# lucidrains/vit-pytorch

Hardware: NVIDIA H100
Metric: images/sec ViT-B/16 224^2 bf16 fwd (higher is better)
Workload: dtype bf16

## Files before the change

### vit_pytorch_b200/csrc/gemm.cu

```cuda
#include "common.cuh"
#include "host_util.h"

namespace b200 {

constexpr int BLOCK_M = 128;
constexpr int BLOCK_K = 64;
constexpr int WGMMA_K = 16;
constexpr int NUM_THREADS = 384;
constexpr int NUM_CONSUMERS = 256;

struct GemmParams {
  int M, N, K;
  int num_m_tiles, num_n_tiles, num_k_blocks;
  int flags;
  __nv_bfloat16* out_bf16;
  float* out_f32;
  long long ldo;
  const float* bias;
  const float* ln_sums;
  int ln_parts;
  int stats_parts;
  int stats_width;
  float ln_inv_dim;
  float ln_eps;
  const float* col_s;
  float* stats_out;
  int rows_per_tile;
  int patch;
  int patch_ght;
  int patch_tiles_per_img;
  int patch_C;
};

template <int BLOCK_N, int STAGES, bool PATCH = false, bool RES = false, bool TMA_OUT = false>
struct GemmSmem {
  static constexpr int A_SLAB = PATCH ? BLOCK_M * 32 : BLOCK_M * BLOCK_K * 2;
  static constexpr int A_BYTES = PATCH ? 4 * A_SLAB : A_SLAB;
  static constexpr int B_BYTES = BLOCK_N * BLOCK_K * 2;
  static constexpr int STAGE_BYTES = A_BYTES + B_BYTES;
  static constexpr int RES_BOX = BLOCK_M * 32 * 4;
  static constexpr int RES_SLAB = 2 * RES_BOX;
  static constexpr int RES_OFFSET = STAGES * STAGE_BYTES;
  static constexpr int OUT_BOX = 64 * 64 * 2;
  static constexpr int OUT_OFFSET = RES_OFFSET + (RES ? 2 * RES_SLAB : 0);
  static constexpr int OUT_BYTES = !TMA_OUT ? 0 : RES ? 2 * OUT_BOX : BLOCK_M * BLOCK_N * 2;
  static constexpr int VEC_OFFSET = OUT_OFFSET + OUT_BYTES;
  static constexpr int VEC_BYTES = (2 * BLOCK_N + 2 * BLOCK_M) * 4;
  static constexpr int BAR_OFFSET = VEC_OFFSET + 2 * VEC_BYTES;
  static constexpr int TOTAL = BAR_OFFSET + (2 * STAGES + 8) * 8;
  static constexpr int DYN_BYTES = TOTAL + 1024;
};

__device__ __forceinline__ void warpgroup_sync(int c) { asm volatile("bar.sync %0, 128;" ::"r"(c + 1) : "memory"); }

template <int BLOCK_N, int STAGES, bool PATCH, bool RES, bool TMA_OUT>
__global__ void __launch_bounds__(NUM_THREADS, 1)
gemm_bf16_kernel(const __grid_constant__ CUtensorMap tmA, const __grid_constant__ CUtensorMap tmB,
                 const __grid_constant__ CUtensorMap tmR, const __grid_constant__ CUtensorMap tmO,
                 const __grid_constant__ CUtensorMap tmF, const GemmParams p) {
  static_assert(!(TMA_OUT && PATCH), "patch tiles have fewer than 128 rows: a 64-row box would overwrite the next one");
  using L = GemmSmem<BLOCK_N, STAGES, PATCH, RES, TMA_OUT>;
  constexpr int NACC = BLOCK_N / 2;
  constexpr int CHUNKS = BLOCK_N / 64;

  extern __shared__ uint8_t smem_raw[];
  uint8_t* smem = smem_raw + ((1024u - (smem_u32(smem_raw) & 1023u)) & 1023u);
  uint64_t* full_bar = reinterpret_cast<uint64_t*>(smem + L::BAR_OFFSET);
  uint64_t* empty_bar = full_bar + STAGES;
  uint64_t* res_full = empty_bar + STAGES;
  uint64_t* res_empty = res_full + 2;
  uint64_t* vec_full = res_empty + 2;
  uint64_t* vec_empty = vec_full + 2;

  const int wg = threadIdx.x >> 7;
  const int num_tiles = p.num_m_tiles * p.num_n_tiles;

  if (threadIdx.x == 0) {
    tma_prefetch_desc(&tmA);
    tma_prefetch_desc(&tmB);
    if (RES) tma_prefetch_desc(&tmR);
    if (TMA_OUT && p.out_bf16) tma_prefetch_desc(&tmO);
    if (TMA_OUT && RES && p.out_f32) tma_prefetch_desc(&tmF);
    for (int s = 0; s < STAGES; ++s) {
      mbar_init(&full_bar[s], 1);
      mbar_init(&empty_bar[s], 2);
    }
    for (int s = 0; s < 2; ++s) {
      mbar_init(&res_full[s], 1);
      mbar_init(&res_empty[s], TMA_OUT ? 2 : NUM_CONSUMERS);
      mbar_init(&vec_full[s], 64);
      mbar_init(&vec_empty[s], NUM_CONSUMERS);
    }
    fence_mbar_init();
  }
  __syncthreads();

  if (wg == 0) {
    setmaxnreg_dec<40>();
    if (threadIdx.x == 0) {
      int stage = 0;
      uint32_t phase = 0;
      for (int tile = blockIdx.x; tile < num_tiles; tile += gridDim.x) {
        const int m_blk = tile / p.num_n_tiles;
        const int n_blk = tile % p.num_n_tiles;
        for (int kb = 0; kb < p.num_k_blocks; ++kb) {
          mbar_wait(&empty_bar[stage], phase ^ 1);
          uint8_t* sa = smem + stage * L::STAGE_BYTES;
          uint8_t* sb = sa + L::A_BYTES;
          if (PATCH) {
            const int img = m_blk / p.patch_tiles_per_img, tin = m_blk % p.patch_tiles_per_img;
            mbar_arrive_expect_tx(&full_bar[stage], p.rows_per_tile * 128 + L::B_BYTES);
#pragma unroll
            for (int j = 0; j < 4; ++j)
              tma_load_5d(sa + j * L::A_SLAB, &tmA, &full_bar[stage], 0, 0, tin * p.patch_ght, (kb & 3) * 4 + j,
                          img * p.patch_C + (kb >> 2));
          } else {
            mbar_arrive_expect_tx(&full_bar[stage], L::STAGE_BYTES);
            tma_load_2d(sa, &tmA, &full_bar[stage], kb * BLOCK_K, m_blk * BLOCK_M);
          }
          tma_load_2d(sb, &tmB, &full_bar[stage], kb * BLOCK_K, n_blk * BLOCK_N);
          if (++stage == STAGES) {
            stage = 0;
            phase ^= 1;
          }
        }
      }
    } else if (RES && threadIdx.x == 32) {
      int it = 0;
      for (int tile = blockIdx.x; tile < num_tiles; tile += gridDim.x) {
        const int n0 = (tile % p.num_n_tiles) * BLOCK_N;
        const int m0 = (tile / p.num_n_tiles) * BLOCK_M;
        const int nslab = min(CHUNKS, (p.N - n0 + 63) / 64);
        for (int q = 0; q < nslab; ++q, ++it) {
          const int buf = it & 1;
          mbar_wait(&res_empty[buf], ((it >> 1) & 1) ^ 1);
          const int c0 = n0 + 64 * q;
          const int nbox = c0 + 32 < p.N ? 2 : 1;
          mbar_arrive_expect_tx(&res_full[buf], nbox * L::RES_BOX);
          uint8_t* slab = smem + L::RES_OFFSET + buf * L::RES_SLAB;
          for (int b = 0; b < nbox; ++b) tma_load_2d(slab + b * L::RES_BOX, &tmR, &res_full[buf], c0 + 32 * b, m0);
        }
      }
    } else if ((threadIdx.x >> 5) >= 2) {
      const int lane = threadIdx.x & 31;
      const bool vec_warp = (threadIdx.x >> 5) == 2;
      int it = 0;
      for (int tile = blockIdx.x; tile < num_tiles; tile += gridDim.x, ++it) {
        const int m_blk = tile / p.num_n_tiles;
        const int n0 = (tile % p.num_n_tiles) * BLOCK_N;
        const int vb = it & 1;
        mbar_wait(&vec_empty[vb], ((it >> 1) & 1) ^ 1);
        float* vbias = reinterpret_cast<float*>(smem + L::VEC_OFFSET + vb * L::VEC_BYTES);
        float* vcs = vbias + BLOCK_N;
        float2* vln = reinterpret_cast<float2*>(vcs + BLOCK_N);
        if (vec_warp) {
#pragma unroll
          for (int i = lane; i < BLOCK_N; i += 32) {
            const int col = n0 + i;
            vbias[i] = (p.flags & B200VIT_EPI_BIAS) && col < p.N ? p.bias[col] : 0.f;
            vcs[i] = (p.flags & B200VIT_EPI_LNFOLD) && col < p.N ? p.col_s[col] : 0.f;
          }
        } else if (p.flags & B200VIT_EPI_LNFOLD) {
          float s1[BLOCK_M / 32], s2[BLOCK_M / 32];
          bool ok[BLOCK_M / 32];
#pragma unroll
          for (int k = 0; k < BLOCK_M / 32; ++k) {
            const int tr = lane + 32 * k;
            ok[k] = m_blk * p.rows_per_tile + tr < p.M && tr < p.rows_per_tile;
            s1[k] = s2[k] = 0.f;
          }
#pragma unroll 1
          for (int i = 0; i < p.ln_parts; ++i)
#pragma unroll
            for (int k = 0; k < BLOCK_M / 32; ++k)
              if (ok[k]) {
                const size_t row = (size_t)m_blk * p.rows_per_tile + lane + 32 * k;
                const float2 ss = *reinterpret_cast<const float2*>(p.ln_sums + 2 * (row * p.ln_parts + i));
                s1[k] += ss.x;
                s2[k] += ss.y;
              }
#pragma unroll
          for (int k = 0; k < BLOCK_M / 32; ++k) vln[lane + 32 * k] = make_float2(s1[k], s2[k]);
        }
        mbar_arrive(&vec_full[vb]);
      }
    }
    return;
  }

  setmaxnreg_inc<232>();
  const int c = wg - 1;
  const int t = threadIdx.x & 127;
  const int warp = t >> 5, lane = t & 31;
  const int flags = p.flags;
  const bool vec_ok = (p.ldo & 1) == 0;
  int stage = 0;
  uint32_t phase = 0;
  int slab_it = 0;
  int pend_slab = -1;
  uint8_t* const stg_wg = smem + L::OUT_OFFSET + c * (RES ? L::OUT_BOX : 64 * BLOCK_N * 2);
  float acc[NACC];

  for (int tile = blockIdx.x, it = 0; tile < num_tiles; tile += gridDim.x, ++it) {
    const int m_blk = tile / p.num_n_tiles;
    const int n_blk = tile % p.num_n_tiles;

    int prev_stage = -1;
    for (int kb = 0; kb < p.num_k_blocks; ++kb) {
      mbar_wait(&full_bar[stage], phase);
      const uint32_t sa = smem_u32(smem + stage * L::STAGE_BYTES);
      const uint32_t sb = sa + L::A_BYTES;
      const uint64_t bdesc = make_wgmma_desc(sb, 1024, WGMMA_SW128);
      wgmma_fence();
#pragma unroll
      for (int k = 0; k < BLOCK_K / WGMMA_K; ++k) {
        const uint64_t ad = PATCH ? make_wgmma_desc(sa + k * L::A_SLAB + c * 64 * 32, 256, WGMMA_SW32)
                                  : make_wgmma_desc(sa + c * 64 * 128, 1024, WGMMA_SW128) + 2 * k;
        if constexpr (BLOCK_N == 256) wgmma_m64n256k16(acc, ad, bdesc + 2 * k, (kb | k) != 0);
        else wgmma_m64n128k16(acc, ad, bdesc + 2 * k, (kb | k) != 0);
      }
      wgmma_commit();
      if (TMA_OUT && kb == 0 && t == 0) {
        tma_store_wait_read<0>();
        if (RES && pend_slab >= 0) mbar_arrive(&res_empty[pend_slab]);
        pend_slab = -1;
      }
      wgmma_wait<1>();
      if (prev_stage >= 0 && t == 0) mbar_arrive(&empty_bar[prev_stage]);
      prev_stage = stage;
      if (++stage == STAGES) {
        stage = 0;
        phase ^= 1;
      }
    }
    wgmma_wait<0>();
    fence_regs(acc);
    if (t == 0) mbar_arrive(&empty_bar[prev_stage]);
    if (TMA_OUT && !RES) warpgroup_sync(c);

    const int tr0 = c * 64 + warp * 16 + (lane >> 2);
    const int vb = it & 1;
    mbar_wait(&vec_full[vb], (it >> 1) & 1);
    const float* vbias = reinterpret_cast<const float*>(smem + L::VEC_OFFSET + vb * L::VEC_BYTES);
    const float* vcs = vbias + BLOCK_N;
    const float2* vln = reinterpret_cast<const float2*>(vcs + BLOCK_N);
    float mu[2] = {0.f, 0.f}, rstd[2] = {1.f, 1.f};
    int row[2];
    bool row_ok[2];
#pragma unroll
    for (int h = 0; h < 2; ++h) {
      const int tr = tr0 + 8 * h;
      row[h] = m_blk * p.rows_per_tile + tr;
      row_ok[h] = row[h] < p.M && tr < p.rows_per_tile;
      if ((flags & B200VIT_EPI_LNFOLD) && row_ok[h]) {
        const float2 ss = vln[tr];
        const float s1 = ss.x, s2 = ss.y;
        mu[h] = s1 * p.ln_inv_dim;
        const float var = fmaxf(s2 * p.ln_inv_dim - mu[h] * mu[h], 0.f);
        rstd[h] = rsqrtf(var + p.ln_eps);
      }
    }
    float st_sum[2][CHUNKS], st_sq[2][CHUNKS];
#pragma unroll
    for (int q = 0; q < CHUNKS; ++q) st_sum[0][q] = st_sum[1][q] = st_sq[0][q] = st_sq[1][q] = 0.f;

    const int n0 = n_blk * BLOCK_N;
    const int nslab = RES ? min(CHUNKS, (p.N - n0 + 63) / 64) : 0;
    const int res_off = tr0 * 128 + (lane & 1) * 8;
    const int res_xor = ((lane & 3) >> 1) ^ (lane >> 2);
    const int stg_off = (tr0 - 64 * c) * 128 + 4 * (lane & 3);
    uint32_t pks[8][2] = {};
#pragma unroll
    for (int j = 0; j < BLOCK_N / 8; ++j) {
      const int pc = 8 * j + 2 * (lane & 3);
      const int col = n0 + pc;
      if (RES && j % 8 == 0 && j / 8 < nslab) mbar_wait(&res_full[slab_it & 1], (slab_it >> 1) & 1);
      uint8_t* slab = smem + L::RES_OFFSET + (slab_it & 1) * L::RES_SLAB + ((j % 8) / 4) * L::RES_BOX + res_off;
      uint8_t* stg = stg_wg + (RES ? 0 : (j / 8) * L::OUT_BOX) + stg_off + (((j % 8) ^ (lane >> 2)) << 4);
      const bool pair = vec_ok && col + 1 < p.N;
      float b0 = 0.f, b1 = 0.f, s0 = 0.f, s1 = 0.f;
      if (flags & B200VIT_EPI_BIAS) {
        const float2 bb = *reinterpret_cast<const float2*>(vbias + pc);
        b0 = bb.x;
        b1 = bb.y;
      }
      if (flags & B200VIT_EPI_LNFOLD) {
        const float2 ss = *reinterpret_cast<const float2*>(vcs + pc);
        s0 = ss.x;
        s1 = ss.y;
      }
#pragma unroll
      for (int h = 0; h < 2; ++h) {
        if (!row_ok[h] || col >= p.N) continue;
        float v0 = acc[4 * j + 2 * h], v1 = acc[4 * j + 2 * h + 1];
        if (flags & (B200VIT_EPI_LNFOLD | B200VIT_EPI_BIAS)) {
          const bool fold = (flags & B200VIT_EPI_LNFOLD) != 0;
          const float k = -rstd[h] * mu[h];
          const float c0 = fold ? fmaf(k, s0, b0) : b0, c1 = fold ? fmaf(k, s1, b1) : b1;
          const float rs = fold ? rstd[h] : 1.0f;
          v0 = fmaf(v0, rs, c0);
          v1 = fmaf(v1, rs, c1);
        }
        if (flags & B200VIT_EPI_GELU) gelu_erf2(v0, v1);
        const size_t o = (size_t)row[h] * p.ldo + col;
        float2* rp = reinterpret_cast<float2*>(slab + h * 8 * 128 + ((((j % 4) * 2) ^ res_xor) << 4));
        float2 rr = make_float2(0.f, 0.f);
        if (RES) rr = *rp;
        float r0 = 0.f, r1 = 0.f;
        if (TMA_OUT) {
          if (RES) {
            v0 += rr.x;
            v1 += rr.y;
            if (p.out_f32) *rp = make_float2(v0, v1);
          }
          const uint32_t pk = pack_bf16x2(v0, v1);
          if (RES) pks[j % 8][h] = pk;
          else *reinterpret_cast<uint32_t*>(stg + h * 8 * 128) = pk;
          r0 = __uint_as_float(pk << 16);
          r1 = __uint_as_float(pk & 0xFFFF0000u);
        } else if (pair) {
          if (RES) {
            v0 += rr.x;
            v1 += rr.y;
          }
          if (p.out_f32) *reinterpret_cast<float2*>(p.out_f32 + o) = make_float2(v0, v1);
          const uint32_t pk = pack_bf16x2(v0, v1);
          if (p.out_bf16) *reinterpret_cast<uint32_t*>(p.out_bf16 + o) = pk;
          r0 = __uint_as_float(pk << 16);
          r1 = __uint_as_float(pk & 0xFFFF0000u);
        } else {
          const float vv[2] = {v0, v1}, res[2] = {rr.x, rr.y};
          float rb[2] = {0.f, 0.f};
          for (int i = 0; i < 2 && col + i < p.N; ++i) {
            float x = vv[i];
            if (RES) x += res[i];
            if (p.out_f32) p.out_f32[o + i] = x;
            const __nv_bfloat16 xb = __float2bfloat16_rn(x);
            if (p.out_bf16) p.out_bf16[o + i] = xb;
            rb[i] = __bfloat162float(xb);
          }
          r0 = rb[0];
          r1 = rb[1];
        }
        if (flags & B200VIT_EPI_STATS) {
          st_sum[h][j / 8] += r0 + r1;
          st_sq[h][j / 8] = fmaf(r0, r0, fmaf(r1, r1, st_sq[h][j / 8]));
        }
      }
      if (RES && j % 8 == 7 && j / 8 < nslab) {
        if constexpr (TMA_OUT) {
          if (t == 0) {
            tma_store_wait_read<0>();
            if (pend_slab >= 0) mbar_arrive(&res_empty[pend_slab]);
            pend_slab = -1;
          }
          warpgroup_sync(c);
          if (p.out_bf16)
#pragma unroll
            for (int jj = 0; jj < 8; ++jj)
#pragma unroll
              for (int h = 0; h < 2; ++h)
                *reinterpret_cast<uint32_t*>(stg_wg + stg_off + ((jj ^ (lane >> 2)) << 4) + h * 8 * 128) = pks[jj][h];
          fence_proxy_async_smem();
          warpgroup_sync(c);
          if (t == 0) {
            const int buf = slab_it & 1, c0 = n0 + 64 * (j / 8), row0 = m_blk * BLOCK_M + 64 * c;
            if (row0 < p.M) {
              const uint8_t* half = smem + L::RES_OFFSET + buf * L::RES_SLAB + c * 64 * 128;
              if (p.out_f32)
                for (int b = 0; b < 2 && c0 + 32 * b < p.N; ++b)
                  tma_store_2d(&tmF, half + b * L::RES_BOX, c0 + 32 * b, row0);
              if (p.out_bf16) tma_store_2d(&tmO, stg_wg, c0, row0);
            }
            tma_store_commit();
            pend_slab = buf;
          }
        } else {
          mbar_arrive(&res_empty[slab_it & 1]);
        }
        ++slab_it;
      }
    }
    mbar_arrive(&vec_empty[vb]);
    if constexpr (TMA_OUT && !RES) {
      fence_proxy_async_smem();
      warpgroup_sync(c);
      if (t == 0) {
        const int row0 = m_blk * BLOCK_M + 64 * c;
        if (row0 < p.M)
          for (int b = 0; b < BLOCK_N / 64 && n0 + 64 * b < p.N; ++b)
            tma_store_2d(&tmO, stg_wg + b * L::OUT_BOX, n0 + 64 * b, row0);
        tma_store_commit();
      }
    }
    if (flags & B200VIT_EPI_STATS) {
#pragma unroll
      for (int h = 0; h < 2; ++h)
#pragma unroll
        for (int q = 0; q < CHUNKS; ++q) {
          st_sum[h][q] += __shfl_xor_sync(0xffffffffu, st_sum[h][q], 1);
          st_sum[h][q] += __shfl_xor_sync(0xffffffffu, st_sum[h][q], 2);
          st_sq[h][q] += __shfl_xor_sync(0xffffffffu, st_sq[h][q], 1);
          st_sq[h][q] += __shfl_xor_sync(0xffffffffu, st_sq[h][q], 2);
        }
      if ((lane & 3) == 0) {
        const int per = p.stats_width / 64;
        const int first = n0 / p.stats_width;
        const int last = (n_blk == p.num_n_tiles - 1) ? p.stats_parts : first + CHUNKS / per;
#pragma unroll
        for (int h = 0; h < 2; ++h) {
          if (!row_ok[h]) continue;
          float* so = p.stats_out + 2 * (size_t)row[h] * p.stats_parts;
          for (int part = first; part < last; ++part) {
            float a = 0.f, b = 0.f;
#pragma unroll
            for (int q = 0; q < CHUNKS; ++q)
              if (first + q / per == part) {
                a += st_sum[h][q];
                b += st_sq[h][q];
              }
            *reinterpret_cast<float2*>(so + 2 * part) = make_float2(a, b);
          }
        }
      }
    }
  }
  if (TMA_OUT && t == 0) tma_store_wait<0>();
}

static std::atomic<int> g_gemm_block_n{0};
void gemm_set_block_n(int v) { g_gemm_block_n = v; }
static std::atomic<int> g_gemm_direct_store{0};
void gemm_set_direct_store(int v) { g_gemm_direct_store = v; }

template <int BLOCK_N, int STAGES, bool PATCH = false, bool RES = false, bool TMA_OUT = false>
static int launch_gemm(const CUtensorMap& tmA, const CUtensorMap& tmB, const CUtensorMap& tmR, const CUtensorMap& tmO,
                       const CUtensorMap& tmF, GemmParams& p, cudaStream_t stream) {
  using L = GemmSmem<BLOCK_N, STAGES, PATCH, RES, TMA_OUT>;
  static_assert(L::DYN_BYTES <= 227 * 1024, "gemm: shared memory budget");
  auto kern = gemm_bf16_kernel<BLOCK_N, STAGES, PATCH, RES, TMA_OUT>;
  B200_ENSURE_SMEM(kern, L::DYN_BYTES);
  if (!p.patch) p.rows_per_tile = BLOCK_M;
  p.num_m_tiles = (p.M + p.rows_per_tile - 1) / p.rows_per_tile;
  p.num_n_tiles = (p.N + BLOCK_N - 1) / BLOCK_N;
  p.num_k_blocks = (p.K + BLOCK_K - 1) / BLOCK_K;
  p.stats_width = p.N > 128 ? 128 : 64;
  const int tiles = p.num_m_tiles * p.num_n_tiles;
  const int grid = tiles < num_sms() ? tiles : num_sms();
  kern<<<grid, NUM_THREADS, L::DYN_BYTES, stream>>>(tmA, tmB, tmR, tmO, tmF, p);
  B200_CHECK_CUDA(cudaGetLastError());
  count_launch();
  return 0;
}

}

extern "C" int b200vit_stats_parts(int N) {
  const int block_n = N > 128 ? 256 : 128;
  return 2 * ((N + block_n - 1) / block_n);
}

extern "C" int b200vit_gemm_bf16(const void* A, int64_t lda, const void* W, int64_t ldw, void* out_bf16,
                                 float* out_f32, int64_t ldo, const float* bias, const float* resid,
                                 const float* ln_sums, int ln_parts, float ln_eps, const float* col_s,
                                 float* stats_out, int M, int N, int K, int flags, void* stream) {
  using namespace b200;
  B200_CHECK_ARG(A && W, "gemm: A/W must not be null");
  B200_CHECK_ARG(out_bf16 || out_f32, "gemm: need at least one output");
  B200_CHECK_ARG(M > 0 && N > 0 && K > 0, "gemm: bad shape M=%d N=%d K=%d", M, N, K);
  B200_CHECK_ARG((reinterpret_cast<uintptr_t>(A) & 15) == 0 && (reinterpret_cast<uintptr_t>(W) & 15) == 0,
                 "gemm: A and W must be 16-byte aligned");
  B200_CHECK_ARG((lda & 7) == 0 && (ldw & 7) == 0 && lda >= K && ldw >= K,
                 "gemm: lda=%lld ldw=%lld must be multiples of 8 and >= K=%d", (long long)lda, (long long)ldw, K);
  B200_CHECK_ARG(ldo >= N, "gemm: ldo=%lld < N=%d", (long long)ldo, N);
  B200_CHECK_ARG(!(flags & B200VIT_EPI_BIAS) || bias, "gemm: EPI_BIAS without bias");
  B200_CHECK_ARG(!(flags & B200VIT_EPI_RESIDUAL) || resid, "gemm: EPI_RESIDUAL without resid");
  B200_CHECK_ARG(!(flags & B200VIT_EPI_RESIDUAL) || (ldo & 3) == 0,
                 "gemm: EPI_RESIDUAL needs ldo=%lld to be a multiple of 4 (16-byte rows for TMA)", (long long)ldo);
  B200_CHECK_ARG(!(flags & B200VIT_EPI_LNFOLD) || (ln_sums && col_s && ln_parts >= 1 && ln_parts <= 64),
                 "gemm: EPI_LNFOLD needs ln_sums, col_s and 1 <= ln_parts <= 64");
  B200_CHECK_ARG(!(flags & B200VIT_EPI_STATS) || stats_out, "gemm: EPI_STATS without stats_out");
  auto al16 = [](const void* q) { return (reinterpret_cast<uintptr_t>(q) & 15) == 0; };
  B200_CHECK_ARG(al16(bias) && al16(resid) && al16(col_s) && al16(out_bf16) && al16(out_f32) && al16(ln_sums),
                 "gemm: epilogue pointers must be 16-byte aligned");

  cudaStream_t st = reinterpret_cast<cudaStream_t>(stream);

  GemmParams p{};
  p.M = M; p.N = N; p.K = K;
  p.flags = flags;
  p.out_bf16 = reinterpret_cast<__nv_bfloat16*>(out_bf16);
  p.out_f32 = out_f32;
  p.ldo = ldo;
  p.bias = bias;
  p.ln_sums = ln_sums;
  p.ln_parts = ln_parts;
  p.stats_parts = b200vit_stats_parts(N);
  p.ln_inv_dim = 1.0f / (float)K;
  p.ln_eps = ln_eps;
  p.col_s = col_s;
  p.stats_out = stats_out;

  const bool res = (flags & B200VIT_EPI_RESIDUAL) != 0;
  const bool tma_ok = !g_gemm_direct_store.load() && ((ldo | N) & 7) == 0 && (res || !out_f32);
  const int force = g_gemm_block_n.load();
  const bool wide = force == 0 ? N > 128 && !(res && tma_ok) : force == 2;
  const uint32_t block_n = wide ? 256 : 128;
  const bool tma_out = tma_ok && !(res && wide);
  CUtensorMap tmA, tmB, tmR{}, tmO{}, tmF{};
  if (tma_out && out_bf16) {
    const uint64_t dims[2] = {(uint64_t)N, (uint64_t)M};
    const uint64_t strides[1] = {(uint64_t)ldo * 2};
    const uint32_t box[2] = {64, 64};
    int rc = encode_tmap_bf16(&tmO, out_bf16, 2, dims, strides, box);
    if (rc) return rc;
  }
  if (tma_out && res && out_f32) {
    const uint64_t dims[2] = {(uint64_t)N, (uint64_t)M};
    const uint64_t strides[1] = {(uint64_t)ldo * 4};
    const uint32_t box[2] = {32, 64};
    int rc = encode_tmap_f32(&tmF, out_f32, 2, dims, strides, box, true);
    if (rc) return rc;
  }
  if (res) {
    const uint64_t dims[2] = {(uint64_t)N, (uint64_t)M};
    const uint64_t strides[1] = {(uint64_t)ldo * 4};
    const uint32_t box[2] = {32, (uint32_t)BLOCK_M};
    int rc = encode_tmap_f32(&tmR, resid, 2, dims, strides, box, true);
    if (rc) return rc;
  }
  {
    const uint64_t dims[2] = {(uint64_t)K, (uint64_t)M};
    const uint64_t strides[1] = {(uint64_t)lda * 2};
    const uint32_t box[2] = {(uint32_t)BLOCK_K, (uint32_t)BLOCK_M};
    int rc = encode_tmap_bf16(&tmA, A, 2, dims, strides, box);
    if (rc) return rc;
  }
  {
    const uint64_t dims[2] = {(uint64_t)K, (uint64_t)N};
    const uint64_t strides[1] = {(uint64_t)ldw * 2};
    const uint32_t box[2] = {(uint32_t)BLOCK_K, block_n};
    int rc = encode_tmap_bf16(&tmB, W, 2, dims, strides, box);
    if (rc) return rc;
  }
  if (tma_out) {
    if (res) return launch_gemm<128, 4, false, true, true>(tmA, tmB, tmR, tmO, tmF, p, st);
    return wide ? launch_gemm<256, 3, false, false, true>(tmA, tmB, tmR, tmO, tmF, p, st)
                : launch_gemm<128, 5, false, false, true>(tmA, tmB, tmR, tmO, tmF, p, st);
  }
  if (wide)
    return res ? launch_gemm<256, 3, false, true>(tmA, tmB, tmR, tmO, tmF, p, st)
               : launch_gemm<256, 4>(tmA, tmB, tmR, tmO, tmF, p, st);
  return res ? launch_gemm<128, 4, false, true>(tmA, tmB, tmR, tmO, tmF, p, st)
             : launch_gemm<128, 6>(tmA, tmB, tmR, tmO, tmF, p, st);
}

extern "C" int b200vit_rmsnorm_heads(void* buf, int64_t ld, const float* gamma, int T, int nheads, int dh, void* stream);
extern "C" int b200vit_layernorm_heads(void* buf, int64_t ld, const float* gamma, int T, int nheads, int dh, float eps,
                                       void* stream);

extern "C" int b200vit_gemm_headnorm_bf16(const void* A, int64_t lda, const void* W, int64_t ldw, void* out_bf16,
                                          int64_t ldo, const float* bias, const float* ln_sums, int ln_parts,
                                          float ln_eps, const float* col_s, const float* head_gamma, int norm_heads,
                                          int dh, float head_eps, int M, int N, int K, int flags, void* stream) {
  using namespace b200;
  B200_CHECK_ARG(out_bf16 && head_gamma, "gemm_headnorm: null pointer");
  B200_CHECK_ARG(head_width_ok(dh), "gemm_headnorm: dim_head=%d not supported by this build (32, 64, 80 or 128)", dh);
  B200_CHECK_ARG(norm_heads > 0 && norm_heads * dh <= N, "gemm_headnorm: %d heads do not fit N=%d", norm_heads, N);
  B200_CHECK_ARG((flags & ~(B200VIT_EPI_BIAS | B200VIT_EPI_LNFOLD | B200VIT_EPI_HEADLN)) == 0,
                 "gemm_headnorm: unsupported flags %d", flags);
  const bool hln = (flags & B200VIT_EPI_HEADLN) != 0;
  B200_CHECK_ARG((reinterpret_cast<uintptr_t>(head_gamma) & 15) == 0, "gemm_headnorm: head_gamma must be 16-byte aligned");
  int rc = b200vit_gemm_bf16(A, lda, W, ldw, out_bf16, nullptr, ldo, bias, nullptr, ln_sums, ln_parts, ln_eps, col_s,
                             nullptr, M, N, K, flags & ~B200VIT_EPI_HEADLN, stream);
  if (rc) return rc;
  if (hln) return b200vit_layernorm_heads(out_bf16, ldo, head_gamma, M, norm_heads, dh, head_eps, stream);
  return b200vit_rmsnorm_heads(out_bf16, ldo, head_gamma, M, norm_heads, dh, stream);
}


extern "C" int b200vit_patch_embed_tma(const void* img, const void* w_perm, const float* bias, const float* col_s,
                                       const float* patch_stats, float ln_eps, float* out_f32, int64_t ldo, int B, int C,
                                       int H, int W, int D, void* stream) {
  using namespace b200;
  B200_CHECK_ARG(img && w_perm && bias && col_s && patch_stats && out_f32, "patch_embed_tma: null pointer");
  B200_CHECK_ARG(B > 0 && C > 0 && C <= 8 && H > 0 && W > 0 && (H % 16) == 0 && (W % 16) == 0,
                 "patch_embed_tma: needs 16 x 16 patches on an image whose sides are multiples of 16 (got %dx%d)", H, W);
  B200_CHECK_ARG(D > 0 && (D % 8) == 0 && ldo >= D, "patch_embed_tma: bad D=%d / ldo", D);
  B200_CHECK_ARG((reinterpret_cast<uintptr_t>(img) & 15) == 0 && (reinterpret_cast<uintptr_t>(w_perm) & 15) == 0 &&
                     (reinterpret_cast<uintptr_t>(out_f32) & 15) == 0 && (reinterpret_cast<uintptr_t>(bias) & 15) == 0 &&
                     (reinterpret_cast<uintptr_t>(col_s) & 15) == 0,
                 "patch_embed_tma: pointers must be 16-byte aligned");
  const int gh = H / 16, gw = W / 16;
  B200_CHECK_ARG(gw <= 128, "patch_embed_tma: %d patches per row do not fit a 128-row tile", gw);
  int ght = 1;
  for (int d = 1; d <= gh; ++d)
    if (gh % d == 0 && d * gw <= 128) ght = d;
  const int K = C * 256;
  GemmParams p{};
  p.M = B * gh * gw; p.N = D; p.K = K;
  p.flags = B200VIT_EPI_LNFOLD | B200VIT_EPI_BIAS;
  p.out_f32 = out_f32;
  p.ldo = ldo;
  p.bias = bias;
  p.ln_sums = patch_stats;
  p.ln_parts = 1;
  p.stats_parts = b200vit_stats_parts(D);
  p.ln_inv_dim = 1.0f / (float)K;
  p.ln_eps = ln_eps;
  p.col_s = col_s;
  p.patch = 1;
  p.patch_ght = ght;
  p.patch_tiles_per_img = gh / ght;
  p.patch_C = C;
  p.rows_per_tile = ght * gw;
  CUtensorMap tmA, tmB, tmR{}, tmO{}, tmF{};
  {
    const uint64_t dims[5] = {16, (uint64_t)gw, (uint64_t)gh, 16, (uint64_t)B * C};
    const uint64_t strides[4] = {32, (uint64_t)16 * W * 2, (uint64_t)W * 2, (uint64_t)H * W * 2};
    const uint32_t box[5] = {16, (uint32_t)gw, (uint32_t)ght, 1, 1};
    int rc = encode_tmap_bf16_sw(&tmA, img, 5, dims, strides, box, 32);
    if (rc) return rc;
  }
  {
    const uint64_t dims[2] = {(uint64_t)K, (uint64_t)D};
    const uint64_t strides[1] = {(uint64_t)K * 2};
    const uint32_t box[2] = {(uint32_t)BLOCK_K, 256};
    int rc = encode_tmap_bf16(&tmB, w_perm, 2, dims, strides, box);
    if (rc) return rc;
  }
  return launch_gemm<256, 4, true>(tmA, tmB, tmR, tmO, tmF, p, reinterpret_cast<cudaStream_t>(stream));
}
```

Before: 10910.

## Overlap residual GEMM epilogue with next tile's mainloop using dual accumulators

Moves the epilogue into a TileEpilogue struct and adds an OVERLAP variant for residual TMA-store GEMMs with at most 16 k-blocks and no LN-fold or GELU. This variant keeps two 64-register accumulator sets, so the previous tile's epilogue runs in chunks while the next tile's first WGMMA k-blocks are issued, hiding epilogue latency behind tensor-core work. The residual path also stops buffering packed bf16 values in registers and writes them straight to the staging buffer, adding a drain/sync at each slab start. The cost is higher register pressure and more complex synchronization, which risks spills or stalls.

```diff
diff --git a/vit_pytorch_b200/csrc/gemm.cu b/vit_pytorch_b200/csrc/gemm.cu
--- a/vit_pytorch_b200/csrc/gemm.cu
+++ b/vit_pytorch_b200/csrc/gemm.cu
@@ -1,3 +1,6 @@
+#include <type_traits>
+#include <utility>
+
 #include "common.cuh"
 #include "host_util.h"
 
@@ -8,6 +11,9 @@
 constexpr int WGMMA_K = 16;
 constexpr int NUM_THREADS = 384;
 constexpr int NUM_CONSUMERS = 256;
+constexpr int EPI_GROUPS = 2;
+constexpr int EPI_STEPS = 128 / 8 / EPI_GROUPS;
+constexpr int OVERLAP_MAX_K_BLOCKS = 16;
 
 struct GemmParams {
   int M, N, K;
@@ -53,12 +59,259 @@
 
 __device__ __forceinline__ void warpgroup_sync(int c) { asm volatile("bar.sync %0, 128;" ::"r"(c + 1) : "memory"); }
 
-template <int BLOCK_N, int STAGES, bool PATCH, bool RES, bool TMA_OUT>
+template <class F, int... S>
+__device__ __forceinline__ void static_for_impl(F& f, std::integer_sequence<int, S...>) {
+  (f(std::integral_constant<int, S>{}), ...);
+}
+template <int N, class F>
+__device__ __forceinline__ void static_for(F&& f) {
+  static_for_impl(f, std::make_integer_sequence<int, N>{});
+}
+
+template <int BLOCK_N, int STAGES, bool PATCH, bool RES, bool TMA_OUT, bool OVERLAP>
+struct TileEpilogue {
+  using L = GemmSmem<BLOCK_N, STAGES, PATCH, RES, TMA_OUT>;
+  static constexpr int NACC = BLOCK_N / 2;
+  static constexpr int CHUNKS = BLOCK_N / 64;
+  static constexpr bool FOLD_GELU = !OVERLAP;
+
+  const GemmParams& p;
+  const CUtensorMap* const tmO;
+  const CUtensorMap* const tmF;
+  uint8_t* const smem;
+  uint64_t* const res_full;
+  uint64_t* const res_empty;
+  uint64_t* const vec_full;
+  uint64_t* const vec_empty;
+  const int c, t, lane;
+  const int tr0;
+  const bool vec_ok;
+  const uint32_t res_x;
+  const uint32_t stg_x;
+  uint8_t* const stg_wg;
+  int slab_it = 0;
+  int pend_slab = -1;
+
+  int m_blk, n_blk, n0, vb, nslab;
+  const float* vbias;
+  const float* vcs;
+  float mu[2], rstd[2];
+  int row0;
+  bool row_ok[2];
+  float st_sum[2][CHUNKS], st_sq[2][CHUNKS];
+
+  __device__ __forceinline__ TileEpilogue(const GemmParams& p_, const CUtensorMap* tmO_, const CUtensorMap* tmF_,
+                                          uint8_t* smem_, uint64_t* res_full_, int c_, int t_)
+      : p(p_), tmO(tmO_), tmF(tmF_), smem(smem_), res_full(res_full_), res_empty(res_full_ + 2), vec_full(res_full_ + 4),
+        vec_empty(res_full_ + 6), c(c_), t(t_), lane(t_ & 31), tr0(c_ * 64 + (t_ >> 5) * 16 + ((t_ & 31) >> 2)),
+        vec_ok((p_.ldo & 1) == 0), res_x(tr0 * 128 + (((lane & 3) >> 1) ^ (lane >> 2)) * 16 + (lane & 1) * 8),
+        stg_x((tr0 - 64 * c_) * 128 + (lane >> 2) * 16 + 4 * (lane & 3)),
+        stg_wg(smem_ + L::OUT_OFFSET + c_ * (RES ? L::OUT_BOX : 64 * BLOCK_N * 2)) {}
+
+  __device__ __forceinline__ void drain() {
+    tma_store_wait_read<0>();
+    if (RES && pend_slab >= 0) mbar_arrive(&res_empty[pend_slab]);
+    pend_slab = -1;
+  }
+
+  __device__ __forceinline__ void begin(int tile, int it) {
+    if constexpr (TMA_OUT) {
+      if (t == 0) drain();
+      if (!RES) warpgroup_sync(c);
+    }
+    m_blk = tile / p.num_n_tiles;
+    n_blk = tile % p.num_n_tiles;
+    row0 = m_blk * p.rows_per_tile + tr0;
+    n0 = n_blk * BLOCK_N;
+    nslab = RES ? min(CHUNKS, (p.N - n0 + 63) / 64) : 0;
+    vb = it & 1;
+    mbar_wait(&vec_full[vb], (it >> 1) & 1);
+    vbias = reinterpret_cast<const float*>(smem + L::VEC_OFFSET + vb * L::VEC_BYTES);
+    vcs = vbias + BLOCK_N;
+    const float2* vln = reinterpret_cast<const float2*>(vcs + BLOCK_N);
+#pragma unroll
+    for (int h = 0; h < 2; ++h) {
+      const int tr = tr0 + 8 * h;
+      mu[h] = 0.f;
+      rstd[h] = 1.f;
+      row_ok[h] = m_blk * p.rows_per_tile + tr < p.M && tr < p.rows_per_tile;
+      if (FOLD_GELU && (p.flags & B200VIT_EPI_LNFOLD) && row_ok[h]) {
+        const float2 ss = vln[tr];
+        const float s1 = ss.x, s2 = ss.y;
+        mu[h] = s1 * p.ln_inv_dim;
+        const float var = fmaxf(s2 * p.ln_inv_dim - mu[h] * mu[h], 0.f);
+        rstd[h] = rsqrtf(var + p.ln_eps);
+      }
+    }
+#pragma unroll
+    for (int q = 0; q < CHUNKS; ++q) st_sum[0][q] = st_sum[1][q] = st_sq[0][q] = st_sq[1][q] = 0.f;
+  }
+
+  template <int J0, int J1>
+  __device__ __forceinline__ void groups(const float (&acc)[NACC]) {
+    const int flags = p.flags;
+    uint32_t rx = res_x, sx = stg_x;
+    asm volatile("" : "+r"(rx), "+r"(sx));
+#pragma unroll
+    for (int j = J0; j < J1; ++j) {
+      const int pc = 8 * j + 2 * (lane & 3);
+      const int col = n0 + pc;
+      if (RES && j % 8 == 0 && j / 8 < nslab) {
+        mbar_wait(&res_full[slab_it & 1], (slab_it >> 1) & 1);
+        if constexpr (TMA_OUT) {
+          if (t == 0) drain();
+          warpgroup_sync(c);
+        }
+      }
+      uint8_t* slab = smem + L::RES_OFFSET + (slab_it & 1) * L::RES_SLAB + ((j % 8) / 4) * L::RES_BOX;
+      uint8_t* stg = stg_wg + (RES ? 0 : (j / 8) * L::OUT_BOX) + (sx ^ ((j % 8) << 4));
+      const bool pair = vec_ok && col + 1 < p.N;
+      float b0 = 0.f, b1 = 0.f, s0 = 0.f, s1 = 0.f;
+      if (flags & B200VIT_EPI_BIAS) {
+        const float2 bb = *reinterpret_cast<const float2*>(vbias + pc);
+        b0 = bb.x;
+        b1 = bb.y;
+      }
+      if (FOLD_GELU && (flags & B200VIT_EPI_LNFOLD)) {
+        const float2 ss = *reinterpret_cast<const float2*>(vcs + pc);
+        s0 = ss.x;
+        s1 = ss.y;
+      }
+#pragma unroll
+      for (int h = 0; h < 2; ++h) {
+        if (!row_ok[h] || col >= p.N) continue;
+        float v0 = acc[4 * j + 2 * h], v1 = acc[4 * j + 2 * h + 1];
+        if (flags & (B200VIT_EPI_LNFOLD | B200VIT_EPI_BIAS)) {
+          const bool fold = FOLD_GELU && (flags & B200VIT_EPI_LNFOLD) != 0;
+          const float k = -rstd[h] * mu[h];
+          const float c0 = fold ? fmaf(k, s0, b0) : b0, c1 = fold ? fmaf(k, s1, b1) : b1;
+          const float rs = fold ? rstd[h] : 1.0f;
+          v0 = fmaf(v0, rs, c0);
+          v1 = fmaf(v1, rs, c1);
+        }
+        if (FOLD_GELU && (flags & B200VIT_EPI_GELU)) gelu_erf2(v0, v1);
+        const size_t o = (size_t)(row0 + 8 * h) * p.ldo + col;
+        float2* rp = reinterpret_cast<float2*>(slab + h * 8 * 128 + (rx ^ (((j % 4) * 2) << 4)));
+        float2 rr = make_float2(0.f, 0.f);
+        if (RES) rr = *rp;
+        float r0 = 0.f, r1 = 0.f;
+        if (TMA_OUT) {
+          if (RES) {
+            v0 += rr.x;
+            v1 += rr.y;
+            if (p.out_f32) *rp = make_float2(v0, v1);
+          }
+          const uint32_t pk = pack_bf16x2(v0, v1);
+          *reinterpret_cast<uint32_t*>(stg + h * 8 * 128) = pk;
+          r0 = __uint_as_float(pk << 16);
+          r1 = __uint_as_float(pk & 0xFFFF0000u);
+        } else if (pair) {
+          if (RES) {
+            v0 += rr.x;
+            v1 += rr.y;
+          }
+          if (p.out_f32) *reinterpret_cast<float2*>(p.out_f32 + o) = make_float2(v0, v1);
+          const uint32_t pk = pack_bf16x2(v0, v1);
+          if (p.out_bf16) *reinterpret_cast<uint32_t*>(p.out_bf16 + o) = pk;
+          r0 = __uint_as_float(pk << 16);
+          r1 = __uint_as_float(pk & 0xFFFF0000u);
+        } else {
+          const float vv[2] = {v0, v1}, res[2] = {rr.x, rr.y};
+          float rb[2] = {0.f, 0.f};
+          for (int i = 0; i < 2 && col + i < p.N; ++i) {
+            float x = vv[i];
+            if (RES) x += res[i];
+            if (p.out_f32) p.out_f32[o + i] = x;
+            const __nv_bfloat16 xb = __float2bfloat16_rn(x);
+            if (p.out_bf16) p.out_bf16[o + i] = xb;
+            rb[i] = __bfloat162float(xb);
+          }
+          r0 = rb[0];
+          r1 = rb[1];
+        }
+        if (flags & B200VIT_EPI_STATS) {
+          st_sum[h][j / 8] += r0 + r1;
+          st_sq[h][j / 8] = fmaf(r0, r0, fmaf(r1, r1, st_sq[h][j / 8]));
+        }
+      }
+      if (RES && j % 8 == 7 && j / 8 < nslab) {
+        if constexpr (TMA_OUT) {
+          fence_proxy_async_smem();
+          warpgroup_sync(c);
+          if (t == 0) {
+            const int buf = slab_it & 1, c0 = n0 + 64 * (j / 8), row0 = m_blk * BLOCK_M + 64 * c;
+            if (row0 < p.M) {
+              const uint8_t* half = smem + L::RES_OFFSET + buf * L::RES_SLAB + c * 64 * 128;
+              if (p.out_f32)
+                for (int b = 0; b < 2 && c0 + 32 * b < p.N; ++b)
+                  tma_store_2d(tmF, half + b * L::RES_BOX, c0 + 32 * b, row0);
+              if (p.out_bf16) tma_store_2d(tmO, stg_wg, c0, row0);
+            }
+            tma_store_commit();
+            pend_slab = buf;
+          }
+        } else {
+          mbar_arrive(&res_empty[slab_it & 1]);
+        }
+        ++slab_it;
+      }
+    }
+  }
+
+  __device__ __forceinline__ void end() {
+    mbar_arrive(&vec_empty[vb]);
+    if constexpr (TMA_OUT && !RES) {
+      fence_proxy_async_smem();
+      warpgroup_sync(c);
+      if (t == 0) {
+        const int row0 = m_blk * BLOCK_M + 64 * c;
+        if (row0 < p.M)
+          for (int b = 0; b < BLOCK_N / 64 && n0 + 64 * b < p.N; ++b)
+            tma_store_2d(tmO, stg_wg + b * L::OUT_BOX, n0 + 64 * b, row0);
+        tma_store_commit();
+      }
+    }
+    if (p.flags & B200VIT_EPI_STATS) {
+#pragma unroll
+      for (int h = 0; h < 2; ++h)
+#pragma unroll
+        for (int q = 0; q < CHUNKS; ++q) {
+          st_sum[h][q] += __shfl_xor_sync(0xffffffffu, st_sum[h][q], 1);
+          st_sum[h][q] += __shfl_xor_sync(0xffffffffu, st_sum[h][q], 2);
+          st_sq[h][q] += __shfl_xor_sync(0xffffffffu, st_sq[h][q], 1);
+          st_sq[h][q] += __shfl_xor_sync(0xffffffffu, st_sq[h][q], 2);
+        }
+      if ((lane & 3) == 0) {
+        const int per = p.stats_width / 64;
+        const int first = n0 / p.stats_width;
+        const int last = (n_blk == p.num_n_tiles - 1) ? p.stats_parts : first + CHUNKS / per;
+#pragma unroll
+        for (int h = 0; h < 2; ++h) {
+          if (!row_ok[h]) continue;
+          float* so = p.stats_out + 2 * (size_t)(row0 + 8 * h) * p.stats_parts;
+          for (int part = first; part < last; ++part) {
+            float a = 0.f, b = 0.f;
+#pragma unroll
+            for (int q = 0; q < CHUNKS; ++q)
+              if (first + q / per == part) {
+                a += st_sum[h][q];
+                b += st_sq[h][q];
+              }
+            *reinterpret_cast<float2*>(so + 2 * part) = make_float2(a, b);
+          }
+        }
+      }
+    }
+  }
+};
+
+template <int BLOCK_N, int STAGES, bool PATCH, bool RES, bool TMA_OUT, bool OVERLAP>
 __global__ void __launch_bounds__(NUM_THREADS, 1)
 gemm_bf16_kernel(const __grid_constant__ CUtensorMap tmA, const __grid_constant__ CUtensorMap tmB,
                  const __grid_constant__ CUtensorMap tmR, const __grid_constant__ CUtensorMap tmO,
                  const __grid_constant__ CUtensorMap tmF, const GemmParams p) {
   static_assert(!(TMA_OUT && PATCH), "patch tiles have fewer than 128 rows: a 64-row box would overwrite the next one");
+  static_assert(!OVERLAP || (TMA_OUT && BLOCK_N == 128), "the overlapped schedule holds two 64-register accumulator sets");
   using L = GemmSmem<BLOCK_N, STAGES, PATCH, RES, TMA_OUT>;
   constexpr int NACC = BLOCK_N / 2;
   constexpr int CHUNKS = BLOCK_N / 64;
@@ -191,241 +444,108 @@
   setmaxnreg_inc<232>();
   const int c = wg - 1;
   const int t = threadIdx.x & 127;
-  const int warp = t >> 5, lane = t & 31;
-  const int flags = p.flags;
-  const bool vec_ok = (p.ldo & 1) == 0;
+  TileEpilogue<BLOCK_N, STAGES, PATCH, RES, TMA_OUT, OVERLAP> epi(p, &tmO, &tmF, smem, res_full, c, t);
   int stage = 0;
   uint32_t phase = 0;
-  int slab_it = 0;
-  int pend_slab = -1;
-  uint8_t* const stg_wg = smem + L::OUT_OFFSET + c * (RES ? L::OUT_BOX : 64 * BLOCK_N * 2);
-  float acc[NACC];
-
-  for (int tile = blockIdx.x, it = 0; tile < num_tiles; tile += gridDim.x, ++it) {
-    const int m_blk = tile / p.num_n_tiles;
-    const int n_blk = tile % p.num_n_tiles;
-
-    int prev_stage = -1;
+  int prev_stage = -1;
+
+  auto issue = [&](float (&acc)[NACC], int kb) {
+    mbar_wait(&full_bar[stage], phase);
+    const uint32_t sa = smem_u32(smem + stage * L::STAGE_BYTES);
+    const uint32_t sb = sa + L::A_BYTES;
+    const uint64_t bdesc = make_wgmma_desc(sb, 1024, WGMMA_SW128);
+    wgmma_fence();
+#pragma unroll
+    for (int k = 0; k < BLOCK_K / WGMMA_K; ++k) {
+      const uint64_t ad = PATCH ? make_wgmma_desc(sa + k * L::A_SLAB + c * 64 * 32, 256, WGMMA_SW32)
+                                : make_wgmma_desc(sa + c * 64 * 128, 1024, WGMMA_SW128) + 2 * k;
+      if constexpr (BLOCK_N == 256) wgmma_m64n256k16(acc, ad, bdesc + 2 * k, (kb | k) != 0);
+      else wgmma_m64n128k16(acc, ad, bdesc + 2 * k, (kb | k) != 0);
+    }
+    wgmma_commit();
+  };
+  auto retire = [&]() {
+    if (prev_stage >= 0 && t == 0) mbar_arrive(&empty_bar[prev_stage]);
+    prev_stage = stage;
+    if (++stage == STAGES) {
+      stage = 0;
+      phase ^= 1;
+    }
+  };
+  auto main_loop = [&](float (&acc)[NACC]) {
+#pragma unroll 1
     for (int kb = 0; kb < p.num_k_blocks; ++kb) {
-      mbar_wait(&full_bar[stage], phase);
-      const uint32_t sa = smem_u32(smem + stage * L::STAGE_BYTES);
-      const uint32_t sb = sa + L::A_BYTES;
-      const uint64_t bdesc = make_wgmma_desc(sb, 1024, WGMMA_SW128);
-      wgmma_fence();
-#pragma unroll
-      for (int k = 0; k < BLOCK_K / WGMMA_K; ++k) {
-        const uint64_t ad = PATCH ? make_wgmma_desc(sa + k * L::A_SLAB + c * 64 * 32, 256, WGMMA_SW32)
-                                  : make_wgmma_desc(sa + c * 64 * 128, 1024, WGMMA_SW128) + 2 * k;
-        if constexpr (BLOCK_N == 256) wgmma_m64n256k16(acc, ad, bdesc + 2 * k, (kb | k) != 0);
-        else wgmma_m64n128k16(acc, ad, bdesc + 2 * k, (kb | k) != 0);
-      }
-      wgmma_commit();
-      if (TMA_OUT && kb == 0 && t == 0) {
-        tma_store_wait_read<0>();
-        if (RES && pend_slab >= 0) mbar_arrive(&res_empty[pend_slab]);
-        pend_slab = -1;
-      }
+      issue(acc, kb);
+      if (RES && TMA_OUT && kb == 0 && t == 0) epi.drain();
       wgmma_wait<1>();
-      if (prev_stage >= 0 && t == 0) mbar_arrive(&empty_bar[prev_stage]);
-      prev_stage = stage;
-      if (++stage == STAGES) {
-        stage = 0;
-        phase ^= 1;
-      }
-    }
+      retire();
+    }
+  };
+  auto finish = [&](float (&acc)[NACC], int tile, int it) {
     wgmma_wait<0>();
     fence_regs(acc);
     if (t == 0) mbar_arrive(&empty_bar[prev_stage]);
-    if (TMA_OUT && !RES) warpgroup_sync(c);
-
-    const int tr0 = c * 64 + warp * 16 + (lane >> 2);
-    const int vb = it & 1;
-    mbar_wait(&vec_full[vb], (it >> 1) & 1);
-    const float* vbias = reinterpret_cast<const float*>(smem + L::VEC_OFFSET + vb * L::VEC_BYTES);
-    const float* vcs = vbias + BLOCK_N;
-    const float2* vln = reinterpret_cast<const float2*>(vcs + BLOCK_N);
-    float mu[2] = {0.f, 0.f}, rstd[2] = {1.f, 1.f};
-    int row[2];
-    bool row_ok[2];
-#pragma unroll
-    for (int h = 0; h < 2; ++h) {
-      const int tr = tr0 + 8 * h;
-      row[h] = m_blk * p.rows_per_tile + tr;
-      row_ok[h] = row[h] < p.M && tr < p.rows_per_tile;
-      if ((flags & B200VIT_EPI_LNFOLD) && row_ok[h]) {
-        const float2 ss = vln[tr];
-        const float s1 = ss.x, s2 = ss.y;
-        mu[h] = s1 * p.ln_inv_dim;
-        const float var = fmaxf(s2 * p.ln_inv_dim - mu[h] * mu[h], 0.f);
-        rstd[h] = rsqrtf(var + p.ln_eps);
-      }
-    }
-    float st_sum[2][CHUNKS], st_sq[2][CHUNKS];
-#pragma unroll
-    for (int q = 0; q < CHUNKS; ++q) st_sum[0][q] = st_sum[1][q] = st_sq[0][q] = st_sq[1][q] = 0.f;
-
-    const int n0 = n_blk * BLOCK_N;
-    const int nslab = RES ? min(CHUNKS, (p.N - n0 + 63) / 64) : 0;
-    const int res_off = tr0 * 128 + (lane & 1) * 8;
-    const int res_xor = ((lane & 3) >> 1) ^ (lane >> 2);
-    const int stg_off = (tr0 - 64 * c) * 128 + 4 * (lane & 3);
-    uint32_t pks[8][2] = {};
-#pragma unroll
-    for (int j = 0; j < BLOCK_N / 8; ++j) {
-      const int pc = 8 * j + 2 * (lane & 3);
-      const int col = n0 + pc;
-      if (RES && j % 8 == 0 && j / 8 < nslab) mbar_wait(&res_full[slab_it & 1], (slab_it >> 1) & 1);
-      uint8_t* slab = smem + L::RES_OFFSET + (slab_it & 1) * L::RES_SLAB + ((j % 8) / 4) * L::RES_BOX + res_off;
-      uint8_t* stg = stg_wg + (RES ? 0 : (j / 8) * L::OUT_BOX) + stg_off + (((j % 8) ^ (lane >> 2)) << 4);
-      const bool pair = vec_ok && col + 1 < p.N;
-      float b0 = 0.f, b1 = 0.f, s0 = 0.f, s1 = 0.f;
-      if (flags & B200VIT_EPI_BIAS) {
-        const float2 bb = *reinterpret_cast<const float2*>(vbias + pc);
-        b0 = bb.x;
-        b1 = bb.y;
-      }
-      if (flags & B200VIT_EPI_LNFOLD) {
-        const float2 ss = *reinterpret_cast<const float2*>(vcs + pc);
-        s0 = ss.x;
-        s1 = ss.y;
-      }
-#pragma unroll
-      for (int h = 0; h < 2; ++h) {
-        if (!row_ok[h] || col >= p.N) continue;
-        float v0 = acc[4 * j + 2 * h], v1 = acc[4 * j + 2 * h + 1];
-        if (flags & (B200VIT_EPI_LNFOLD | B200VIT_EPI_BIAS)) {
-          const bool fold = (flags & B200VIT_EPI_LNFOLD) != 0;
-          const float k = -rstd[h] * mu[h];
-          const float c0 = fold ? fmaf(k, s0, b0) : b0, c1 = fold ? fmaf(k, s1, b1) : b1;
-          const float rs = fold ? rstd[h] : 1.0f;
-          v0 = fmaf(v0, rs, c0);
-          v1 = fmaf(v1, rs, c1);
-        }
-        if (flags & B200VIT_EPI_GELU) gelu_erf2(v0, v1);
-        const size_t o = (size_t)row[h] * p.ldo + col;
-        float2* rp = reinterpret_cast<float2*>(slab + h * 8 * 128 + ((((j % 4) * 2) ^ res_xor) << 4));
-        float2 rr = make_float2(0.f, 0.f);
-        if (RES) rr = *rp;
-        float r0 = 0.f, r1 = 0.f;
-        if (TMA_OUT) {
-          if (RES) {
-            v0 += rr.x;
-            v1 += rr.y;
-            if (p.out_f32) *rp = make_float2(v0, v1);
-          }
-          const uint32_t pk = pack_bf16x2(v0, v1);
-          if (RES) pks[j % 8][h] = pk;
-          else *reinterpret_cast<uint32_t*>(stg + h * 8 * 128) = pk;
-          r0 = __uint_as_float(pk << 16);
-          r1 = __uint_as_float(pk & 0xFFFF0000u);
-        } else if (pair) {
-          if (RES) {
-            v0 += rr.x;
-            v1 += rr.y;
-          }
-          if (p.out_f32) *reinterpret_cast<float2*>(p.out_f32 + o) = make_float2(v0, v1);
-          const uint32_t pk = pack_bf16x2(v0, v1);
-          if (p.out_bf16) *reinterpret_cast<uint32_t*>(p.out_bf16 + o) = pk;
-          r0 = __uint_as_float(pk << 16);
-          r1 = __uint_as_float(pk & 0xFFFF0000u);
-        } else {
-          const float vv[2] = {v0, v1}, res[2] = {rr.x, rr.y};
-          float rb[2] = {0.f, 0.f};
-          for (int i = 0; i < 2 && col + i < p.N; ++i) {
-            float x = vv[i];
-            if (RES) x += res[i];
-            if (p.out_f32) p.out_f32[o + i] = x;
-            const __nv_bfloat16 xb = __float2bfloat16_rn(x);
-            if (p.out_bf16) p.out_bf16[o + i] = xb;
-            rb[i] = __bfloat162float(xb);
-          }
-          r0 = rb[0];
-          r1 = rb[1];
-        }
-        if (flags & B200VIT_EPI_STATS) {
-          st_sum[h][j / 8] += r0 + r1;
-          st_sq[h][j / 8] = fmaf(r0, r0, fmaf(r1, r1, st_sq[h][j / 8]));
-        }
-      }
-      if (RES && j % 8 == 7 && j / 8 < nslab) {
-        if constexpr (TMA_OUT) {
-          if (t == 0) {
-            tma_store_wait_read<0>();
-            if (pend_slab >= 0) mbar_arrive(&res_empty[pend_slab]);
-            pend_slab = -1;
-          }
-          warpgroup_sync(c);
-          if (p.out_bf16)
-#pragma unroll
-            for (int jj = 0; jj < 8; ++jj)
-#pragma unroll
-              for (int h = 0; h < 2; ++h)
-                *reinterpret_cast<uint32_t*>(stg_wg + stg_off + ((jj ^ (lane >> 2)) << 4) + h * 8 * 128) = pks[jj][h];
-          fence_proxy_async_smem();
-          warpgroup_sync(c);
-          if (t == 0) {
-            const int buf = slab_it & 1, c0 = n0 + 64 * (j / 8), row0 = m_blk * BLOCK_M + 64 * c;
-            if (row0 < p.M) {
-              const uint8_t* half = smem + L::RES_OFFSET + buf * L::RES_SLAB + c * 64 * 128;
-              if (p.out_f32)
-                for (int b = 0; b < 2 && c0 + 32 * b < p.N; ++b)
-                  tma_store_2d(&tmF, half + b * L::RES_BOX, c0 + 32 * b, row0);
-              if (p.out_bf16) tma_store_2d(&tmO, stg_wg, c0, row0);
-            }
-            tma_store_commit();
-            pend_slab = buf;
-          }
-        } else {
-          mbar_arrive(&res_empty[slab_it & 1]);
-        }
-        ++slab_it;
-      }
-    }
-    mbar_arrive(&vec_empty[vb]);
-    if constexpr (TMA_OUT && !RES) {
-      fence_proxy_async_smem();
-      warpgroup_sync(c);
-      if (t == 0) {
-        const int row0 = m_blk * BLOCK_M + 64 * c;
-        if (row0 < p.M)
-          for (int b = 0; b < BLOCK_N / 64 && n0 + 64 * b < p.N; ++b)
-            tma_store_2d(&tmO, stg_wg + b * L::OUT_BOX, n0 + 64 * b, row0);
-        tma_store_commit();
-      }
-    }
-    if (flags & B200VIT_EPI_STATS) {
-#pragma unroll
-      for (int h = 0; h < 2; ++h)
-#pragma unroll
-        for (int q = 0; q < CHUNKS; ++q) {
-          st_sum[h][q] += __shfl_xor_sync(0xffffffffu, st_sum[h][q], 1);
-          st_sum[h][q] += __shfl_xor_sync(0xffffffffu, st_sum[h][q], 2);
-          st_sq[h][q] += __shfl_xor_sync(0xffffffffu, st_sq[h][q], 1);
-          st_sq[h][q] += __shfl_xor_sync(0xffffffffu, st_sq[h][q], 2);
-        }
-      if ((lane & 3) == 0) {
-        const int per = p.stats_width / 64;
-        const int first = n0 / p.stats_width;
-        const int last = (n_blk == p.num_n_tiles - 1) ? p.stats_parts : first + CHUNKS / per;
-#pragma unroll
-        for (int h = 0; h < 2; ++h) {
-          if (!row_ok[h]) continue;
-          float* so = p.stats_out + 2 * (size_t)row[h] * p.stats_parts;
-          for (int part = first; part < last; ++part) {
-            float a = 0.f, b = 0.f;
-#pragma unroll
-            for (int q = 0; q < CHUNKS; ++q)
-              if (first + q / per == part) {
-                a += st_sum[h][q];
-                b += st_sq[h][q];
-              }
-            *reinterpret_cast<float2*>(so + 2 * part) = make_float2(a, b);
-          }
-        }
-      }
-    }
-  }
-  if (TMA_OUT && t == 0) tma_store_wait<0>();
+    prev_stage = -1;
+    epi.begin(tile, it);
+    epi.template groups<0, BLOCK_N / 8>(acc);
+    epi.end();
+  };
+
+  if constexpr (!OVERLAP) {
+    float acc[NACC];
+    for (int tile = blockIdx.x, it = 0; tile < num_tiles; tile += gridDim.x, ++it) {
+      main_loop(acc);
+      finish(acc, tile, it);
+    }
+    if (TMA_OUT && t == 0) tma_store_wait<0>();
+  } else {
+    auto main_loop_with_epilogue = [&](float (&acc)[NACC], float (&prev)[NACC], int ptile, int it) {
+      const int nkb = p.num_k_blocks;
+      static_for<EPI_STEPS>([&](auto step) {
+        constexpr int S = decltype(step)::value;
+        if (S < nkb) issue(acc, S);
+        if constexpr (S == 0) {
+          wgmma_wait<1>();
+          fence_regs(prev);
+          retire();
+          epi.begin(ptile, it);
+        }
+        epi.template groups<S * EPI_GROUPS, (S + 1) * EPI_GROUPS>(prev);
+        if constexpr (S == EPI_STEPS - 1) epi.end();
+        if (S > 0 && S < nkb) {
+          wgmma_wait<1>();
+          retire();
+        }
+      });
+#pragma unroll 1
+      for (int kb = EPI_STEPS; kb < nkb; ++kb) {
+        issue(acc, kb);
+        if (RES && kb == EPI_STEPS && t == 0) epi.drain();
+        wgmma_wait<1>();
+        retire();
+      }
+    };
+    float acc0[NACC], acc1[NACC];
+    int tile = blockIdx.x;
+    if (tile < num_tiles) {
+      main_loop(acc0);
+      for (int it = 0;; it += 2) {
+        if (tile + (int)gridDim.x >= num_tiles) {
+          finish(acc0, tile, it);
+          break;
+        }
+        main_loop_with_epilogue(acc1, acc0, tile, it);
+        tile += gridDim.x;
+        if (tile + (int)gridDim.x >= num_tiles) {
+          finish(acc1, tile, it + 1);
+          break;
+        }
+        main_loop_with_epilogue(acc0, acc1, tile, it + 1);
+        tile += gridDim.x;
+      }
+    }
+    if (t == 0) tma_store_wait<0>();
+  }
 }
 
 static std::atomic<int> g_gemm_block_n{0};
@@ -433,12 +553,12 @@
 static std::atomic<int> g_gemm_direct_store{0};
 void gemm_set_direct_store(int v) { g_gemm_direct_store = v; }
 
-template <int BLOCK_N, int STAGES, bool PATCH = false, bool RES = false, bool TMA_OUT = false>
+template <int BLOCK_N, int STAGES, bool PATCH = false, bool RES = false, bool TMA_OUT = false, bool OVERLAP = false>
 static int launch_gemm(const CUtensorMap& tmA, const CUtensorMap& tmB, const CUtensorMap& tmR, const CUtensorMap& tmO,
                        const CUtensorMap& tmF, GemmParams& p, cudaStream_t stream) {
   using L = GemmSmem<BLOCK_N, STAGES, PATCH, RES, TMA_OUT>;
   static_assert(L::DYN_BYTES <= 227 * 1024, "gemm: shared memory budget");
-  auto kern = gemm_bf16_kernel<BLOCK_N, STAGES, PATCH, RES, TMA_OUT>;
+  auto kern = gemm_bf16_kernel<BLOCK_N, STAGES, PATCH, RES, TMA_OUT, OVERLAP>;
   B200_ENSURE_SMEM(kern, L::DYN_BYTES);
   if (!p.patch) p.rows_per_tile = BLOCK_M;
   p.num_m_tiles = (p.M + p.rows_per_tile - 1) / p.rows_per_tile;
@@ -544,6 +664,9 @@
     if (rc) return rc;
   }
   if (tma_out) {
+    if (res && (K + BLOCK_K - 1) / BLOCK_K <= OVERLAP_MAX_K_BLOCKS &&
+        !(flags & (B200VIT_EPI_LNFOLD | B200VIT_EPI_GELU)))
+      return launch_gemm<128, 4, false, true, true, true>(tmA, tmB, tmR, tmO, tmF, p, st);
     if (res) return launch_gemm<128, 4, false, true, true>(tmA, tmB, tmR, tmO, tmF, p, st);
     return wide ? launch_gemm<256, 3, false, false, true>(tmA, tmB, tmR, tmO, tmF, p, st)
                 : launch_gemm<128, 5, false, false, true>(tmA, tmB, tmR, tmO, tmF, p, st);
```

After: 11050, median of 6. 1.3% higher.
